# ufal/neuralmonkey

Measured on NVIDIA H100. Metric: train_target_tokens_per_sec, higher is better.
Workload: dtype f32 storage; tensor-core products in fp16 (vocabulary) / tf32 with fp32 accumulation

## Files before the change

neuralmonkey_b200/csrc/gru.cu:

```cuda
#include <stdlib.h>
#include <string.h>

#include "gemm_simt.cuh"
#include "gru_cluster.cuh"

namespace nm {

struct GruGatesEpi {
  const float* xproj;
  const float* hprev;
  float* gates;
  float* rh;
  int64_t T, H, t;
  __device__ void operator()(int64_t b, int64_t n, float acc) const {
    const int64_t base3 = (b * T + t) * 3 * H;
    const float g = sigmoidf_(acc + xproj[base3 + n]);
    gates[base3 + n] = g;
    if (n < H) rh[(b * T + t) * H + n] = g * hprev[(b * T + t) * H + n];
  }
};

struct GruCandEpi {
  const float* xproj;
  const float* hprev;
  float* gates;
  float* states;
  float* hnext;
  int64_t hnext_stride;
  const int32_t* lengths;
  const float* drop_mask;
  float* raw_states;
  int64_t T, H, t;
  __device__ void operator()(int64_t b, int64_t n, float acc) const {
    const int64_t base3 = (b * T + t) * 3 * H;
    const float c = tanhf(acc + xproj[base3 + 2 * H + n]);
    gates[base3 + 2 * H + n] = c;
    const float u = gates[base3 + H + n];
    const float h = hprev[(b * T + t) * H + n];
    const bool live = (lengths == nullptr) || (t < (int64_t)lengths[b]);
    float hn = live ? (u * h + (1.f - u) * c) : h;
    if (raw_states) raw_states[(b * T + t) * H + n] = live ? hn : 0.f;
    if (drop_mask && live) hn *= drop_mask[(b * T + t) * H + n];
    states[(b * T + t) * H + n] = live ? hn : 0.f;
    hnext[b * hnext_stride + n] = hn;
  }
};

__global__ void gru_bwd_gate_kernel(const float* __restrict__ gates, const float* __restrict__ hprev,
                                    const float* __restrict__ dstates, const float* __restrict__ dcarry,
                                    const int32_t* __restrict__ lengths,
                                    const float* __restrict__ drop_mask,
                                    const float* __restrict__ draw, float* __restrict__ dxproj,
                                    float* __restrict__ dhp, int64_t B, int64_t T, int64_t H,
                                    int64_t t) {
  const int64_t total = B * H;
  for (int64_t i = blockIdx.x * (int64_t)blockDim.x + threadIdx.x; i < total;
       i += (int64_t)gridDim.x * blockDim.x) {
    const int64_t b = i / H, n = i - b * H;
    const int64_t base3 = (b * T + t) * 3 * H, base1 = (b * T + t) * H;
    const bool live = (lengths == nullptr) || (t < (int64_t)lengths[b]);
    const float u = gates[base3 + H + n], c = gates[base3 + 2 * H + n];
    const float h = hprev[base1 + n];
    float dh = dcarry ? dcarry[i] : 0.f;
    if (!live) {
      dxproj[base3 + n] = 0.f;
      dxproj[base3 + H + n] = 0.f;
      dxproj[base3 + 2 * H + n] = 0.f;
      dhp[i] = dh;
      continue;
    }
    if (dstates) dh += dstates[base1 + n];
    if (drop_mask) dh *= drop_mask[base1 + n];
    if (draw) dh += draw[base1 + n];
    const float du = dh * (h - c);
    const float dc = dh * (1.f - u);
    dxproj[base3 + 2 * H + n] = dc * (1.f - c * c);
    dxproj[base3 + H + n] = du * u * (1.f - u);
    dhp[i] = dh * u;
  }
}

struct GruBwdCandEpi {
  const float* gates;
  const float* hprev;
  const int32_t* lengths;
  float* dxproj;
  float* dhp;
  int64_t T, H, t;
  __device__ void operator()(int64_t b, int64_t n, float drh) const {
    const bool live = (lengths == nullptr) || (t < (int64_t)lengths[b]);
    if (!live) return;
    const int64_t base3 = (b * T + t) * 3 * H;
    const float r = gates[base3 + n];
    const float h = hprev[(b * T + t) * H + n];
    dxproj[base3 + n] = drh * h * r * (1.f - r);
    dhp[b * H + n] += drh * r;
  }
};

struct GruBwdGatesEpi {
  const float* dhp;
  float* dcarry;
  int64_t H;
  __device__ void operator()(int64_t b, int64_t n, float acc) const {
    dcarry[b * H + n] = dhp[b * H + n] + acc;
  }
};

}

using namespace nm;

namespace {

bool cluster_path_ok(int64_t H) {
  static int forced = -1;
  if (forced < 0) {
    const char* e = getenv("NMB200_GRU");
    forced = (e && strcmp(e, "steps") == 0) ? 1 : 0;
  }
  return forced == 0 && H >= 8 && H <= 320;
}

int g_gru_mode = 0;

struct ClusterPlan {
  int Bc, nclusters, sl;
  size_t smem;
};

template <class Kern>
int max_active_clusters(Kern kern, size_t smem) {
  cudaLaunchConfig_t cfg = {};
  cfg.gridDim = dim3(GC_CLUSTER * 64);
  cfg.blockDim = dim3(GC_THREADS);
  cfg.dynamicSmemBytes = smem;
  cudaLaunchAttribute attr[1];
  attr[0].id = cudaLaunchAttributeClusterDimension;
  attr[0].val.clusterDim.x = GC_CLUSTER;
  attr[0].val.clusterDim.y = 1;
  attr[0].val.clusterDim.z = 1;
  cfg.attrs = attr;
  cfg.numAttrs = 1;
  int n = 0;
  if (cudaFuncSetAttribute(kern, cudaFuncAttributeMaxDynamicSharedMemorySize, GC_SMEM_CAP) != cudaSuccess ||
      cudaOccupancyMaxActiveClusters(&n, kern, &cfg) != cudaSuccess || n < 1) {
    cudaGetLastError();
    n = sm_count() / GC_CLUSTER / 2;
  }
  return n;
}

int resident_clusters(bool backward) {
  static int cached[2] = {0, 0};
  if (cached[backward] == 0)
    cached[backward] = backward ? max_active_clusters(gru_seq_bwd_cluster_kernel<GC_MAX_SL>, 128 * 1024)
                                : max_active_clusters(gru_seq_fwd_cluster_kernel<GC_MAX_SL>, 128 * 1024);
  return cached[backward];
}

ClusterPlan plan_clusters(int64_t B, int64_t H, int sm_budget, bool backward) {
  ClusterPlan p;
  p.sl = (int)((H + GC_SLICES - 1) / GC_SLICES);
  int max_clusters = resident_clusters(backward);
  if (sm_budget > 0 && sm_budget / GC_CLUSTER < max_clusters) max_clusters = sm_budget / GC_CLUSTER;
  if (max_clusters < 1) max_clusters = 1;
  int Bc = (int)((B + max_clusters - 1) / max_clusters);
  Bc = (Bc + 3) / 4 * 4;
  const size_t per_row = (size_t)(backward ? gc_bwd_row_floats(p.sl) : gc_fwd_row_floats(p.sl)) * 4;
  const int cap = (int)((GC_SMEM_CAP - GC_BAR_BYTES) / per_row) / 4 * 4;
  if (Bc > cap) Bc = cap;
  if (Bc < 4) Bc = 4;
  p.Bc = Bc;
  p.nclusters = (int)((B + Bc - 1) / Bc);
  p.smem = GC_BAR_BYTES + per_row * Bc;
  return p;
}

template <class Args, class Kern>
int launch_cluster(Kern kern, const Args& args, const ClusterPlan& p, cudaStream_t s, const char* name) {
  NM_CUDA_TRY(cudaFuncSetAttribute(kern, cudaFuncAttributeMaxDynamicSharedMemorySize, (int)p.smem));
  cudaLaunchConfig_t cfg = {};
  cfg.gridDim = dim3((unsigned)(p.nclusters * GC_CLUSTER));
  cfg.blockDim = dim3(GC_THREADS);
  cfg.dynamicSmemBytes = p.smem;
  cfg.stream = s;
  cudaLaunchAttribute attr[1];
  attr[0].id = cudaLaunchAttributeClusterDimension;
  attr[0].val.clusterDim.x = GC_CLUSTER;
  attr[0].val.clusterDim.y = 1;
  attr[0].val.clusterDim.z = 1;
  cfg.attrs = attr;
  cfg.numAttrs = 1;
  NM_CUDA_TRY(cudaLaunchKernelEx(&cfg, kern, args));
  NM_LAUNCH_CHECK(name);
  return NM_OK;
}

#define NM_GC_DISPATCH(KERN, args, plan, s, name)                  \
  switch ((plan).sl) {                                             \
    case 1: return launch_cluster(KERN<1>, args, plan, s, name);   \
    case 2: return launch_cluster(KERN<2>, args, plan, s, name);   \
    case 3: return launch_cluster(KERN<3>, args, plan, s, name);   \
    case 4: return launch_cluster(KERN<4>, args, plan, s, name);   \
    case 5: return launch_cluster(KERN<5>, args, plan, s, name);   \
    case 6: return launch_cluster(KERN<6>, args, plan, s, name);   \
    case 7: return launch_cluster(KERN<7>, args, plan, s, name);   \
    case 8: return launch_cluster(KERN<8>, args, plan, s, name);   \
    case 9: return launch_cluster(KERN<9>, args, plan, s, name);   \
    default: return launch_cluster(KERN<10>, args, plan, s, name); \
  }

}

extern "C" {

int nm_gru_resident_clusters(int backward) { return resident_clusters(backward != 0); }

int nm_gru_set_mode(int mode) {
  NM_REQUIRE(mode == 0 || mode == 1, NM_E_INVALID, "nm_gru_set_mode: mode must be 0 (tensor cores) or 1 (exact fp32)");
  g_gru_mode = mode;
  return NM_OK;
}

static long long* g_gru_prof = nullptr;
int nm_gru_debug_profile(void* counters) {
  g_gru_prof = reinterpret_cast<long long*>(counters);
  return NM_OK;
}

int nm_gru_seq_fwd(const float* xproj, const float* Wgh, const float* Wch, const float* h0,
                   const int32_t* lengths, const float* drop_mask, int reverse, float* states,
                   float* raw_states, float* final_state, float* gates, float* hprev, float* rh,
                   int64_t B, int64_t T, int64_t H, int sm_budget, void* stream) {
  NM_REQUIRE(xproj && Wgh && Wch && states && final_state && gates && hprev && rh, NM_E_INVALID,
             "nm_gru_seq_fwd: null pointer");
  NM_REQUIRE(B > 0 && T > 0 && H > 0, NM_E_INVALID, "nm_gru_seq_fwd: bad sizes B=%lld T=%lld H=%lld",
             (long long)B, (long long)T, (long long)H);
  cudaStream_t s = (cudaStream_t)stream;
  if (cluster_path_ok(H)) {
    GcFwdArgs a{xproj, Wgh, Wch, h0, lengths, drop_mask, states, raw_states, final_state, gates,
                hprev, rh, (int)B, (int)T, (int)H, 0, reverse, g_gru_prof};
    const ClusterPlan p = plan_clusters(B, H, sm_budget, false);
    a.Bc = p.Bc;
    NM_GC_DISPATCH(gru_seq_fwd_cluster_kernel, a, p, s, "nm_gru_seq_fwd(cluster)");
  }
  const int64_t t_first = reverse ? T - 1 : 0;
  if (h0)
    NM_CUDA_TRY(cudaMemcpy2DAsync(hprev + t_first * H, sizeof(float) * T * H, h0, sizeof(float) * H,
                                  sizeof(float) * H, B, cudaMemcpyDeviceToDevice, s));
  else
    NM_CUDA_TRY(cudaMemset2DAsync(hprev + t_first * H, sizeof(float) * T * H, 0, sizeof(float) * H, B, s));
  for (int64_t step = 0; step < T; ++step) {
    const int64_t t = reverse ? T - 1 - step : step;
    GruGatesEpi e1{xproj, hprev, gates, rh, T, H, t};
    simt_gemm_launch(hprev + t * H, T * H, 1, Wgh, 2 * H, 1, B, 2 * H, H, e1, s);
    const bool last = (step == T - 1);
    const int64_t t_next = reverse ? t - 1 : t + 1;
    GruCandEpi e2{xproj, hprev, gates, states, last ? final_state : hprev + t_next * H,
                  last ? H : T * H, lengths, drop_mask, raw_states, T, H, t};
    simt_gemm_launch(rh + t * H, T * H, 1, Wch, H, 1, B, H, H, e2, s);
  }
  count_launches(2 * T - 1);
  NM_LAUNCH_CHECK("nm_gru_seq_fwd");
  return NM_OK;
}

int nm_gru_seq_bwd(const float* Wgh, const float* Wch, const int32_t* lengths,
                   const float* drop_mask, int reverse, const float* gates, const float* hprev,
                   const float* dstates, const float* draw, const float* dfinal,
                   float* dxproj, float* dh0, float* work, int64_t B, int64_t T, int64_t H,
                   int sm_budget, void* stream) {
  NM_REQUIRE(Wgh && Wch && gates && hprev && dxproj && work, NM_E_INVALID,
             "nm_gru_seq_bwd: null pointer");
  NM_REQUIRE(B > 0 && T > 0 && H > 0, NM_E_INVALID, "nm_gru_seq_bwd: bad sizes");
  cudaStream_t s = (cudaStream_t)stream;
  if (cluster_path_ok(H)) {
    GcBwdArgs a{Wgh, Wch, lengths, drop_mask, gates, hprev, dstates, draw, dfinal, dxproj, dh0,
                (int)B, (int)T, (int)H, 0, reverse, g_gru_prof};
    const ClusterPlan p = plan_clusters(B, H, sm_budget, true);
    a.Bc = p.Bc;
    NM_GC_DISPATCH(gru_seq_bwd_cluster_kernel, a, p, s, "nm_gru_seq_bwd(cluster)");
  }
  float* dcarry = work;
  float* dhp = work + B * H;
  if (dfinal)
    NM_CUDA_TRY(cudaMemcpyAsync(dcarry, dfinal, sizeof(float) * B * H, cudaMemcpyDeviceToDevice, s));
  else
    NM_CUDA_TRY(cudaMemsetAsync(dcarry, 0, sizeof(float) * B * H, s));
  const int threads = 256;
  int64_t blocks = ceil_div(B * H, threads);
  const int64_t cap = (int64_t)sm_count() * 8;
  if (blocks > cap) blocks = cap;
  for (int64_t step = T - 1; step >= 0; --step) {
    const int64_t t = reverse ? T - 1 - step : step;
    gru_bwd_gate_kernel<<<(unsigned)blocks, threads, 0, s>>>(gates, hprev, dstates, dcarry, lengths,
                                                            drop_mask, draw, dxproj, dhp, B, T, H, t);
    GruBwdCandEpi g1{gates, hprev, lengths, dxproj, dhp, T, H, t};
    simt_gemm_launch(dxproj + t * 3 * H + 2 * H, T * 3 * H, 1, Wch, 1, H, B, H, H, g1, s);
    GruBwdGatesEpi g2{dhp, dcarry, H};
    simt_gemm_launch(dxproj + t * 3 * H, T * 3 * H, 1, Wgh, 1, 2 * H, B, H, 2 * H, g2, s);
  }
  if (dh0)
    NM_CUDA_TRY(cudaMemcpyAsync(dh0, dcarry, sizeof(float) * B * H, cudaMemcpyDeviceToDevice, s));
  count_launches(3 * T - 1);
  NM_LAUNCH_CHECK("nm_gru_seq_bwd");
  return NM_OK;
}


int nm_gru_seq_fwd_pair(const float* xproj_a, const float* Wgh_a, const float* Wch_a, int reverse_a,
                        float* states_a, float* final_a, float* gates_a, float* hprev_a, float* rh_a,
                        const float* xproj_b, const float* Wgh_b, const float* Wch_b, int reverse_b,
                        float* states_b, float* final_b, float* gates_b, float* hprev_b, float* rh_b,
                        const int32_t* lengths, int64_t B, int64_t T, int64_t H, void* stream) {
  NM_REQUIRE(xproj_a && Wgh_a && Wch_a && states_a && final_a && gates_a && hprev_a && rh_a && xproj_b &&
                 Wgh_b && Wch_b && states_b && final_b && gates_b && hprev_b && rh_b,
             NM_E_INVALID, "nm_gru_seq_fwd_pair: null pointer");
  NM_REQUIRE(B > 0 && T > 0 && H > 0, NM_E_INVALID, "nm_gru_seq_fwd_pair: bad sizes");
  int rc = nm_gru_seq_fwd(xproj_a, Wgh_a, Wch_a, nullptr, lengths, nullptr, reverse_a, states_a, nullptr, final_a,
                          gates_a, hprev_a, rh_a, B, T, H, 0, stream);
  if (rc) return rc;
  return nm_gru_seq_fwd(xproj_b, Wgh_b, Wch_b, nullptr, lengths, nullptr, reverse_b, states_b, nullptr, final_b,
                        gates_b, hprev_b, rh_b, B, T, H, 0, stream);
}

int nm_gru_seq_bwd_pair(const float* Wgh_a, const float* Wch_a, int reverse_a, const float* gates_a,
                        const float* hprev_a, const float* dstates_a, const float* dfinal_a, float* dxproj_a,
                        const float* Wgh_b, const float* Wch_b, int reverse_b, const float* gates_b,
                        const float* hprev_b, const float* dstates_b, const float* dfinal_b, float* dxproj_b,
                        const int32_t* lengths, float* work, int64_t B, int64_t T, int64_t H, void* stream) {
  NM_REQUIRE(Wgh_a && Wch_a && gates_a && hprev_a && dxproj_a && Wgh_b && Wch_b && gates_b && hprev_b &&
                 dxproj_b && work,
             NM_E_INVALID, "nm_gru_seq_bwd_pair: null pointer");
  NM_REQUIRE(B > 0 && T > 0 && H > 0, NM_E_INVALID, "nm_gru_seq_bwd_pair: bad sizes");
  int rc = nm_gru_seq_bwd(Wgh_a, Wch_a, lengths, nullptr, reverse_a, gates_a, hprev_a, dstates_a, nullptr, dfinal_a,
                          dxproj_a, nullptr, work, B, T, H, 0, stream);
  if (rc) return rc;
  return nm_gru_seq_bwd(Wgh_b, Wch_b, lengths, nullptr, reverse_b, gates_b, hprev_b, dstates_b, nullptr, dfinal_b,
                        dxproj_b, nullptr, work, B, T, H, 0, stream);
}

}
```

neuralmonkey_b200/csrc/gru_cluster.cuh:

```cuda
#pragma once
#include "common.cuh"

namespace nm {

constexpr int GC_CLUSTER = 8;
constexpr int GC_SLICES = 32;
constexpr int GC_UPW = 4;
constexpr int GC_WARPS = 10;
constexpr int GC_THREADS = GC_WARPS * 32;
constexpr int GC_MAX_UNITS = GC_WARPS * GC_UPW;
constexpr int GC_RB = 2;
constexpr int GC_MAX_SL = 10;
constexpr int GC_SMEM_CAP = 200 * 1024;
constexpr int GC_BAR_BYTES = 64;
constexpr int GC_XS = 4;
constexpr int GC_PF = 8;

__host__ __device__ constexpr int gc_row(int SL) { return GC_SLICES * 4 * (((SL + 3) / 4) | 1); }
__host__ __device__ constexpr int gc_fwd_row_floats(int SL) {
  return 3 * gc_row(SL) + GC_MAX_UNITS * (1 + 2 * GC_XS) + 1;
}
__host__ __device__ constexpr int gc_bwd_row_floats(int SL) {
  return 4 * gc_row(SL) + GC_MAX_UNITS * (1 + 2 * GC_PF) + 1;
}

template <int SL>
struct GcGeom {
  static constexpr int SLP = 4 * (((SL + 3) / 4) | 1);
  static constexpr int ROW = GC_SLICES * SLP;
  static __device__ __forceinline__ int pos(int j) { return (j / SL) * SLP + (j % SL); }
};

__device__ __forceinline__ void cluster_barrier() {
  asm volatile("barrier.cluster.arrive.release.aligned;\n\tbarrier.cluster.wait.acquire.aligned;" ::
                   : "memory");
}
__device__ __forceinline__ uint32_t cluster_rank() {
  uint32_t r;
  asm volatile("mov.u32 %0, %%cluster_ctarank;" : "=r"(r));
  return r;
}

__device__ __forceinline__ uint32_t gc_smem_u32(const void* p) {
  return (uint32_t)__cvta_generic_to_shared(p);
}
__device__ __forceinline__ void gc_mbar_init(uint32_t bar) {
  asm volatile("mbarrier.init.shared::cta.b64 [%0], 1;" ::"r"(bar));
  asm volatile("fence.mbarrier_init.release.cluster;" ::: "memory");
}
__device__ __forceinline__ void gc_mbar_arm(uint32_t bar, uint32_t bytes) {
  asm volatile("mbarrier.arrive.expect_tx.shared::cta.b64 _, [%0], %1;" ::"r"(bar), "r"(bytes) : "memory");
}
__device__ __forceinline__ void gc_mbar_wait(uint32_t bar, uint32_t parity) {
  uint32_t done;
  do {
    asm volatile(
        "{\n\t.reg .pred p;\n\t"
        "mbarrier.try_wait.parity.acquire.cluster.shared::cta.b64 p, [%1], %2;\n\t"
        "selp.u32 %0, 1, 0, p;\n\t}"
        : "=r"(done)
        : "r"(bar), "r"(parity)
        : "memory");
  } while (!done);
}
__device__ __forceinline__ void gc_send(uint32_t addr, uint32_t bar, uint32_t dst, float v) {
  uint32_t ra, rb;
  asm volatile("mapa.shared::cluster.u32 %0, %1, %2;" : "=r"(ra) : "r"(addr), "r"(dst));
  asm volatile("mapa.shared::cluster.u32 %0, %1, %2;" : "=r"(rb) : "r"(bar), "r"(dst));
  asm volatile("st.async.shared::cluster.mbarrier::complete_tx::bytes.b32 [%0], %1, [%2];" ::"r"(ra),
               "r"(__float_as_uint(v)), "r"(rb)
               : "memory");
}

__device__ __forceinline__ void cp_async4(float* smem_dst, const float* gmem_src) {
  const uint32_t d = gc_smem_u32(smem_dst);
  asm volatile("cp.async.ca.shared.global [%0], [%1], 4;" ::"r"(d), "l"(gmem_src) : "memory");
}
__device__ __forceinline__ void cp_async_commit() { asm volatile("cp.async.commit_group;" ::: "memory"); }
__device__ __forceinline__ void cp_async_wait_all() { asm volatile("cp.async.wait_all;" ::: "memory"); }

template <int N, int O>
__device__ __forceinline__ void gc_reduce_level(float (&v)[N], int lane) {
  constexpr int n = N * O / 16;
  if constexpr (n > 1) {
    const bool upper = (lane & O) != 0;
#pragma unroll
    for (int i = 0; i < n / 2; ++i) {
      const float keep = upper ? v[i + n / 2] : v[i];
      const float send = upper ? v[i] : v[i + n / 2];
      v[i] = keep + __shfl_xor_sync(0xffffffffu, send, O);
    }
  } else {
    v[0] += __shfl_xor_sync(0xffffffffu, v[0], O);
  }
  if constexpr (O > 1) gc_reduce_level<N, O / 2>(v, lane);
}
template <int N>
__device__ __forceinline__ void gc_reduce_scatter(float (&v)[N], int lane) {
  gc_reduce_level<N, 16>(v, lane);
}

template <int SL>
__device__ __forceinline__ void gc_dot(const float* __restrict__ vec, int row0, int lane,
                                       const float (&w)[GC_UPW][SL], float (&acc)[GC_RB][GC_UPW]) {
#pragma unroll
  for (int r = 0; r < GC_RB; ++r)
#pragma unroll
    for (int u = 0; u < GC_UPW; ++u) acc[r][u] = 0.f;
  const float* base = vec + row0 * GcGeom<SL>::ROW + lane * GcGeom<SL>::SLP;
#pragma unroll
  for (int c = 0; c < SL; c += 4) {
    const int n = SL - c < 4 ? SL - c : 4;
#pragma unroll
    for (int r = 0; r < GC_RB; ++r) {
      const float* p = base + r * GcGeom<SL>::ROW + c;
      float x[4];
      if (n == 4) {
        const float4 q = *reinterpret_cast<const float4*>(p);
        x[0] = q.x; x[1] = q.y; x[2] = q.z; x[3] = q.w;
      } else {
        if (n >= 2) {
          const float2 q = *reinterpret_cast<const float2*>(p);
          x[0] = q.x; x[1] = q.y;
        }
        if (n == 1) x[0] = p[0];
        if (n == 3) x[2] = p[2];
      }
#pragma unroll
      for (int u = 0; u < GC_UPW; ++u)
#pragma unroll
        for (int i = 0; i < 4; ++i)
          if (i < n) acc[r][u] = fmaf(x[i], w[u][c + i], acc[r][u]);
    }
  }
}

template <int SL>
__device__ __forceinline__ void gc_load_w(float (&w)[GC_UPW][SL], const float* __restrict__ W,
                                          int64_t sk, int64_t su, int unit0, int unit_limit, int k0, int H) {
#pragma unroll
  for (int u = 0; u < GC_UPW; ++u)
#pragma unroll
    for (int i = 0; i < SL; ++i) {
      const int unit = unit0 + u, k = k0 + i;
      const bool ok = (unit < unit_limit) && (k < H);
      w[u][i] = ok ? W[(int64_t)k * sk + (int64_t)unit * su] : 0.f;
    }
}

struct GcProf {
  bool on;
  unsigned t0;
  __device__ __forceinline__ explicit GcProf(const long long* out)
      : on(out != nullptr && blockIdx.x == 0 && threadIdx.x == 0), t0(on ? (unsigned)clock() : 0u) {}
  __device__ __forceinline__ void lap(long long* out, int slot) {
    if (on) {
      const unsigned t1 = (unsigned)clock();
      out[slot] += (long long)(t1 - t0);
      t0 = t1;
    }
  }
};

struct GcFwdArgs {
  const float* xproj;
  const float* Wgh;
  const float* Wch;
  const float* h0;
  const int32_t* lengths;
  const float* drop_mask;
  float* states;
  float* raw_states;
  float* final_state;
  float* gates;
  float* hprev;
  float* rh;
  int B, T, H, Bc, reverse;
  long long* prof;
};

__device__ __forceinline__ void gc_fwd_prefetch(const GcFwdArgs& a, int t, float* dst, int b0, int nrows,
                                                int ubeg, int UW) {
  const int H = a.H, T = a.T;
  for (int idx = threadIdx.x; idx < a.Bc * UW; idx += GC_THREADS) {
    const int b = idx / UW, ul = idx - b * UW, j = ubeg + ul;
    if (b < nrows && j < H) {
      const int64_t row = ((int64_t)(b0 + b) * T + t);
      const float* xp = a.xproj + row * 3 * H + j;
      float* xd = dst + (b * GC_MAX_UNITS + ul) * GC_XS;
      cp_async4(xd, xp);
      cp_async4(xd + 1, xp + H);
      cp_async4(xd + 2, xp + 2 * H);
      if (a.drop_mask) cp_async4(xd + 3, a.drop_mask + row * H + j);
    }
  }
  cp_async_commit();
}

__device__ __forceinline__ uint32_t gc_phase_bytes(const GcFwdArgs& a) { return (uint32_t)(a.Bc * a.H * 4); }

template <int SL>
__global__ void __launch_bounds__(GC_THREADS, 1) gru_seq_fwd_cluster_kernel(GcFwdArgs a) {
  extern __shared__ __align__(16) float gc_smem[];
  constexpr int ROW = GcGeom<SL>::ROW;
  const int H = a.H, T = a.T, Bc = a.Bc;
  float* hbuf = gc_smem + GC_BAR_BYTES / 4;
  float* rhbuf = hbuf + 2 * Bc * ROW;
  float* us = rhbuf + Bc * ROW;
  float* xs = us + Bc * GC_MAX_UNITS;
  int* lens = reinterpret_cast<int*>(xs + 2 * Bc * GC_MAX_UNITS * GC_XS);
  const uint32_t bar_h = gc_smem_u32(gc_smem), bar_rh = bar_h + 16;

  const int rank = (int)cluster_rank();
  const int ubeg = rank * H / GC_CLUSTER;
  const int unit_limit = (rank + 1) * H / GC_CLUSTER;
  const int UW = unit_limit - ubeg;
  const int b0 = (blockIdx.x / GC_CLUSTER) * Bc;
  const int nrows = min(Bc, a.B - b0);
  const int lane = threadIdx.x & 31, warp = threadIdx.x >> 5;
  const int unit0_local = warp * GC_UPW;
  const int unit0 = ubeg + unit0_local;
  const bool warp_live = unit0 < unit_limit;

  float wr[GC_UPW][SL], wu[GC_UPW][SL], wc[GC_UPW][SL];
  gc_load_w<SL>(wr, a.Wgh, 2 * H, 1, unit0, unit_limit, lane * SL, H);
  gc_load_w<SL>(wu, a.Wgh + H, 2 * H, 1, unit0, unit_limit, lane * SL, H);
  gc_load_w<SL>(wc, a.Wch, H, 1, unit0, unit_limit, lane * SL, H);

  const int g1 = lane >> 4, r1 = (lane >> 3) & 1, u1 = (lane >> 1) & 3;
  const int r2 = (lane >> 4) & 1, u2 = (lane >> 2) & 3, copy2 = lane & 3;
  const int copy1 = ((lane >> 4) << 1) | (lane & 1);
  const bool ok1 = unit0 + u1 < unit_limit, ok2 = unit0 + u2 < unit_limit;
  const int j1 = unit0 + u1, j2 = unit0 + u2;
  const int pos1 = ok1 ? GcGeom<SL>::pos(j1) : 0, pos2 = ok2 ? GcGeom<SL>::pos(j2) : 0;

  if (threadIdx.x == 0) {
    gc_mbar_init(bar_h);
    gc_mbar_init(bar_h + 8);
    gc_mbar_init(bar_rh);
    gc_mbar_arm(bar_h, gc_phase_bytes(a));
    gc_mbar_arm(bar_h + 8, gc_phase_bytes(a));
    gc_mbar_arm(bar_rh, gc_phase_bytes(a));
  }
  for (int i = threadIdx.x; i < 3 * Bc * ROW; i += GC_THREADS) hbuf[i] = 0.f;
  for (int i = threadIdx.x; i < 2 * Bc * GC_MAX_UNITS * GC_XS; i += GC_THREADS) xs[i] = 0.f;
  for (int b = threadIdx.x; b < Bc; b += GC_THREADS)
    lens[b] = b < nrows ? (a.lengths ? a.lengths[b0 + b] : T) : 0;


  __syncthreads();
  cluster_barrier();
  const int t_first = a.reverse ? T - 1 : 0;
  for (int idx = threadIdx.x; idx < Bc * UW; idx += GC_THREADS) {
    const int b = idx / UW, j = ubeg + (idx - b * UW);
    const float hv = (b < nrows && a.h0) ? a.h0[(int64_t)(b0 + b) * H + j] : 0.f;
    if (b < nrows) a.hprev[((int64_t)(b0 + b) * T + t_first) * H + j] = hv;
    const uint32_t addr = gc_smem_u32(hbuf + b * ROW + GcGeom<SL>::pos(j));
    for (int d = 0; d < GC_CLUSTER; ++d) gc_send(addr, bar_h, d, hv);
  }
  gc_fwd_prefetch(a, t_first, xs, b0, nrows, ubeg, UW);

  GcProf prof(a.prof);
  for (int step = 0; step < T; ++step) {
    const int t = a.reverse ? T - 1 - step : step;
    const bool last = (step == T - 1);
    const int t_next = a.reverse ? t - 1 : t + 1;
    const int64_t row0 = (int64_t)b0 * T + t;
    const int par = step & 1;
    const float* hb = hbuf + par * Bc * ROW;
    const float* xc = xs + par * Bc * GC_MAX_UNITS * GC_XS;

    gc_mbar_wait(bar_h + 8 * par, (step >> 1) & 1);
    if (threadIdx.x == 0 && step + 2 < T) gc_mbar_arm(bar_h + 8 * par, gc_phase_bytes(a));
    prof.lap(a.prof, 0);
    cp_async_wait_all();
    __syncthreads();
    if (!last) gc_fwd_prefetch(a, t_next, xs + (par ^ 1) * Bc * GC_MAX_UNITS * GC_XS, b0, nrows, ubeg, UW);
    prof.lap(a.prof, 1);

    if (warp_live) {
      for (int r0 = 0; r0 < Bc; r0 += GC_RB) {
        float ar[GC_RB][GC_UPW], au[GC_RB][GC_UPW];
        gc_dot<SL>(hb, r0, lane, wr, ar);
        gc_dot<SL>(hb, r0, lane, wu, au);
        float v[2 * GC_RB * GC_UPW];
#pragma unroll
        for (int r = 0; r < GC_RB; ++r)
#pragma unroll
          for (int u = 0; u < GC_UPW; ++u) {
            v[r * GC_UPW + u] = ar[r][u];
            v[GC_RB * GC_UPW + r * GC_UPW + u] = au[r][u];
          }
        gc_reduce_scatter<2 * GC_RB * GC_UPW>(v, lane);
        const int b = r0 + r1, ul = unit0_local + u1;
        const float g = sigmoidf_(v[0] + xc[(b * GC_MAX_UNITS + ul) * GC_XS + g1]);
        const float rhv = g * hb[b * ROW + pos1];
        const float rh_peer = __shfl_xor_sync(0xffffffffu, rhv, 16);
        const float rh_send = g1 == 0 ? rhv : rh_peer;
        if (ok1) {
          if ((lane & 1) == 0) {
            if (b < nrows) {
              const int64_t row = row0 + (int64_t)b * T;
              a.gates[row * 3 * H + g1 * H + j1] = g;
              if (g1 == 0) a.rh[row * H + j1] = rhv;
            }
            if (g1 == 1) us[b * GC_MAX_UNITS + ul] = g;
          }
          const uint32_t addr = gc_smem_u32(rhbuf + b * ROW + pos1);
          gc_send(addr, bar_rh, 2 * copy1, rh_send);
          gc_send(addr, bar_rh, 2 * copy1 + 1, rh_send);
        }
      }
      __syncwarp();
    }
    prof.lap(a.prof, 2);
    gc_mbar_wait(bar_rh, step & 1);
    if (threadIdx.x == 0 && !last) gc_mbar_arm(bar_rh, gc_phase_bytes(a));
    prof.lap(a.prof, 3);

    if (warp_live) {
      const uint32_t bar_next = bar_h + 8 * (par ^ 1);
      float* hn_buf = hbuf + (par ^ 1) * Bc * ROW;
      for (int r0 = 0; r0 < Bc; r0 += GC_RB) {
        float ac[GC_RB][GC_UPW];
        gc_dot<SL>(rhbuf, r0, lane, wc, ac);
        float v[GC_RB * GC_UPW];
#pragma unroll
        for (int r = 0; r < GC_RB; ++r)
#pragma unroll
          for (int u = 0; u < GC_UPW; ++u) v[r * GC_UPW + u] = ac[r][u];
        gc_reduce_scatter<GC_RB * GC_UPW>(v, lane);
        if (!ok2) continue;
        const int b = r0 + r2, ul = unit0_local + u2;
        const float* xd = xc + (b * GC_MAX_UNITS + ul) * GC_XS;
        const float c = tanhf(v[0] + xd[2]);
        const float hv = hb[b * ROW + pos2];
        const float uu = us[b * GC_MAX_UNITS + ul];
        const bool live = t < lens[b];
        float hn = live ? (uu * hv + (1.f - uu) * c) : hv;
        const float raw = live ? hn : 0.f;
        if (a.drop_mask && live) hn *= xd[3];
        if (b < nrows) {
          const int64_t row = row0 + (int64_t)b * T;
          if (copy2 == 0) a.gates[row * 3 * H + 2 * H + j2] = c;
          else if (copy2 == 1) a.states[row * H + j2] = live ? hn : 0.f;
          else if (copy2 == 2) { if (a.raw_states) a.raw_states[row * H + j2] = raw; }
          else if (last) a.final_state[(int64_t)(b0 + b) * H + j2] = hn;
          else a.hprev[((int64_t)(b0 + b) * T + t_next) * H + j2] = hn;
        }
        if (!last) {
          const uint32_t addr = gc_smem_u32(hn_buf + b * ROW + pos2);
          gc_send(addr, bar_next, 2 * copy2, hn);
          gc_send(addr, bar_next, 2 * copy2 + 1, hn);
        }
      }
    }
    prof.lap(a.prof, 4);
  }
  cluster_barrier();
}

struct GcBwdArgs {
  const float* Wgh;
  const float* Wch;
  const int32_t* lengths;
  const float* drop_mask;
  const float* gates;
  const float* hprev;
  const float* dstates;
  const float* draw;
  const float* dfinal;
  float* dxproj;
  float* dh0;
  int B, T, H, Bc, reverse;
  long long* prof;
};

__device__ __forceinline__ float gc_bwd_e1(const GcBwdArgs& a, const float* pf, float dh, bool live,
                                           float& zc, float& zu) {
  if (!live) {
    zc = zu = 0.f;
    return dh;
  }
  const float uu = pf[1], c = pf[2], hv = pf[3];
  if (a.dstates) dh += pf[4];
  if (a.drop_mask) dh *= pf[5];
  if (a.draw) dh += pf[6];
  const float du = dh * (hv - c);
  const float dc = dh * (1.f - uu);
  zc = dc * (1.f - c * c);
  zu = du * uu * (1.f - uu);
  return dh * uu;
}

__device__ __forceinline__ void gc_bwd_prefetch(const GcBwdArgs& a, int t, float* dst, const int* lens, int b0,
                                                int ubeg, int UW) {
  const int H = a.H, T = a.T;
  for (int idx = threadIdx.x; idx < a.Bc * UW; idx += GC_THREADS) {
    const int b = idx / UW, u = idx - b * UW, j = ubeg + u;
    if (t >= lens[b]) continue;
    const int64_t row = (int64_t)(b0 + b) * T + t;
    float* d = dst + (b * GC_MAX_UNITS + u) * GC_PF;
    const float* g = a.gates + row * 3 * H + j;
    cp_async4(d, g);
    cp_async4(d + 1, g + H);
    cp_async4(d + 2, g + 2 * H);
    cp_async4(d + 3, a.hprev + row * H + j);
    if (a.dstates) cp_async4(d + 4, a.dstates + row * H + j);
    if (a.drop_mask) cp_async4(d + 5, a.drop_mask + row * H + j);
    if (a.draw) cp_async4(d + 6, a.draw + row * H + j);
  }
  cp_async_commit();
}

template <int SL>
__global__ void __launch_bounds__(GC_THREADS, 1) gru_seq_bwd_cluster_kernel(GcBwdArgs a) {
  extern __shared__ __align__(16) float gc_smem[];
  constexpr int ROW = GcGeom<SL>::ROW;
  const int H = a.H, T = a.T, Bc = a.Bc;
  float* vc = gc_smem + GC_BAR_BYTES / 4;
  float* vu = vc + Bc * ROW;
  float* vr = vu + 2 * Bc * ROW;
  float* dhp = vr + Bc * ROW;
  float* pf = dhp + Bc * GC_MAX_UNITS;
  int* lens = reinterpret_cast<int*>(pf + 2 * Bc * GC_MAX_UNITS * GC_PF);
  const uint32_t bar_a = gc_smem_u32(gc_smem), bar_b = bar_a + 16;
  const uint32_t bytes_a = (uint32_t)(2 * Bc * H * 4), bytes_b = (uint32_t)(Bc * H * 4);

  const int rank = (int)cluster_rank();
  const int ubeg = rank * H / GC_CLUSTER;
  const int unit_limit = (rank + 1) * H / GC_CLUSTER;
  const int UW = unit_limit - ubeg;
  const int b0 = (blockIdx.x / GC_CLUSTER) * Bc;
  const int nrows = min(Bc, a.B - b0);
  const int lane = threadIdx.x & 31, warp = threadIdx.x >> 5;
  const int unit0_local = warp * GC_UPW;
  const int unit0 = ubeg + unit0_local;
  const bool warp_live = unit0 < unit_limit;

  float w1[GC_UPW][SL], w2r[GC_UPW][SL], w2u[GC_UPW][SL];
  gc_load_w<SL>(w1, a.Wch, 1, H, unit0, unit_limit, lane * SL, H);
  gc_load_w<SL>(w2r, a.Wgh, 1, 2 * H, unit0, unit_limit, lane * SL, H);
  gc_load_w<SL>(w2u, a.Wgh + H, 1, 2 * H, unit0, unit_limit, lane * SL, H);

  const int rr_ = (lane >> 4) & 1, uq = (lane >> 2) & 3, copy = lane & 3;
  const bool ok = unit0 + uq < unit_limit;
  const int ji = unit0 + uq, ul = unit0_local + uq;
  const int pos = ok ? GcGeom<SL>::pos(ji) : 0;
  auto time_of = [reverse = a.reverse, T](int k) { return reverse ? k : T - 1 - k; };

  if (threadIdx.x == 0) {
    gc_mbar_init(bar_a);
    gc_mbar_init(bar_a + 8);
    gc_mbar_init(bar_b);
    gc_mbar_arm(bar_a, bytes_a);
    gc_mbar_arm(bar_a + 8, bytes_a);
    gc_mbar_arm(bar_b, bytes_b);
  }
  for (int i = threadIdx.x; i < 4 * Bc * ROW; i += GC_THREADS) vc[i] = 0.f;
  for (int i = threadIdx.x; i < 2 * Bc * GC_MAX_UNITS * GC_PF; i += GC_THREADS) pf[i] = 0.f;
  for (int b = threadIdx.x; b < Bc; b += GC_THREADS)
    lens[b] = b < nrows ? (a.lengths ? a.lengths[b0 + b] : T) : 0;
  __syncthreads();


  gc_bwd_prefetch(a, time_of(0), pf, lens, b0, ubeg, UW);
  cp_async_wait_all();
  __syncthreads();
  cluster_barrier();
  {
    const int t = time_of(0);
    for (int idx = threadIdx.x; idx < Bc * UW; idx += GC_THREADS) {
      const int b = idx / UW, u = idx - b * UW, j = ubeg + u;
      const bool live = t < lens[b];
      const float dh = (a.dfinal && b < nrows) ? a.dfinal[(int64_t)(b0 + b) * H + j] : 0.f;
      float zc, zu;
      dhp[b * GC_MAX_UNITS + u] = gc_bwd_e1(a, pf + (b * GC_MAX_UNITS + u) * GC_PF, dh, live, zc, zu);
      if (b < nrows) {
        const int64_t row = (int64_t)(b0 + b) * T + t;
        a.dxproj[row * 3 * H + H + j] = zu;
        a.dxproj[row * 3 * H + 2 * H + j] = zc;
      }
      const int p = GcGeom<SL>::pos(j);
      const uint32_t ac = gc_smem_u32(vc + b * ROW + p), au = gc_smem_u32(vu + b * ROW + p);
      for (int d = 0; d < GC_CLUSTER; ++d) {
        gc_send(ac, bar_a, d, zc);
        gc_send(au, bar_a, d, zu);
      }
    }
  }

  GcProf prof(a.prof);
  for (int k = 0; k < T; ++k) {
    const int t = time_of(k);
    const bool last = (k == T - 1);
    const int64_t row0 = (int64_t)b0 * T + t;
    const int par = k & 1;
    const float* pfc = pf + par * Bc * GC_MAX_UNITS * GC_PF;
    float* pfn = pf + (par ^ 1) * Bc * GC_MAX_UNITS * GC_PF;

    gc_mbar_wait(bar_a + 8 * par, (k >> 1) & 1);
    if (threadIdx.x == 0 && k + 2 < T) gc_mbar_arm(bar_a + 8 * par, bytes_a);
    prof.lap(a.prof, 0);
    __syncthreads();
    if (!last) gc_bwd_prefetch(a, time_of(k + 1), pfn, lens, b0, ubeg, UW);
    prof.lap(a.prof, 1);

    if (warp_live) {
      for (int r0 = 0; r0 < Bc; r0 += GC_RB) {
        float acc[GC_RB][GC_UPW];
        gc_dot<SL>(vc, r0, lane, w1, acc);
        float v[GC_RB * GC_UPW];
#pragma unroll
        for (int r = 0; r < GC_RB; ++r)
#pragma unroll
          for (int u = 0; u < GC_UPW; ++u) v[r * GC_UPW + u] = acc[r][u];
        gc_reduce_scatter<GC_RB * GC_UPW>(v, lane);
        if (!ok) continue;
        const int b = r0 + rr_;
        const float drh = v[0];
        const bool live = t < lens[b];
        const float* s = pfc + (b * GC_MAX_UNITS + ul) * GC_PF;
        const float rg = s[0], hv = s[3];
        const float zr = live ? drh * hv * rg * (1.f - rg) : 0.f;
        if (copy == 0) {
          if (b < nrows) a.dxproj[(row0 + (int64_t)b * T) * 3 * H + ji] = zr;
          if (live) dhp[b * GC_MAX_UNITS + ul] += drh * rg;
        }
        const uint32_t addr = gc_smem_u32(vr + b * ROW + pos);
        gc_send(addr, bar_b, 2 * copy, zr);
        gc_send(addr, bar_b, 2 * copy + 1, zr);
      }
      __syncwarp();
    }
    prof.lap(a.prof, 2);
    gc_mbar_wait(bar_b, k & 1);
    if (threadIdx.x == 0 && !last) gc_mbar_arm(bar_b, bytes_b);
    prof.lap(a.prof, 3);
    cp_async_wait_all();
    __syncthreads();
    prof.lap(a.prof, 4);

    if (warp_live) {
      const float* vuc = vu + par * Bc * ROW;
      const int tn = last ? t : time_of(k + 1);
      for (int r0 = 0; r0 < Bc; r0 += GC_RB) {
        float accr[GC_RB][GC_UPW], accu[GC_RB][GC_UPW];
        gc_dot<SL>(vr, r0, lane, w2r, accr);
        gc_dot<SL>(vuc, r0, lane, w2u, accu);
        float v[GC_RB * GC_UPW];
#pragma unroll
        for (int r = 0; r < GC_RB; ++r)
#pragma unroll
          for (int u = 0; u < GC_UPW; ++u) v[r * GC_UPW + u] = accr[r][u] + accu[r][u];
        gc_reduce_scatter<GC_RB * GC_UPW>(v, lane);
        const int b = r0 + rr_;
        const float dcarry = ok ? dhp[b * GC_MAX_UNITS + ul] + v[0] : 0.f;
        __syncwarp();
        if (!ok) continue;
        if (last) {
          if (a.dh0 && copy == 0 && b < nrows) a.dh0[(int64_t)(b0 + b) * H + ji] = dcarry;
          continue;
        }
        float zc, zu;
        const float d = gc_bwd_e1(a, pfn + (b * GC_MAX_UNITS + ul) * GC_PF, dcarry, tn < lens[b], zc, zu);
        if (b < nrows) {
          const int64_t row = (int64_t)(b0 + b) * T + tn;
          if (copy == 1) a.dxproj[row * 3 * H + H + ji] = zu;
          else if (copy == 2) a.dxproj[row * 3 * H + 2 * H + ji] = zc;
        }
        if (copy == 0) dhp[b * GC_MAX_UNITS + ul] = d;
        const uint32_t ac = gc_smem_u32(vc + b * ROW + pos);
        const uint32_t au = gc_smem_u32(vu + ((par ^ 1) * Bc + b) * ROW + pos);
        const uint32_t bar_next = bar_a + 8 * (par ^ 1);
        gc_send(ac, bar_next, 2 * copy, zc);
        gc_send(ac, bar_next, 2 * copy + 1, zc);
        gc_send(au, bar_next, 2 * copy, zu);
        gc_send(au, bar_next, 2 * copy + 1, zu);
      }
    }
    prof.lap(a.prof, 5);
  }
  cluster_barrier();
}

}
```

Before: 1.016 million.

## Stage update-gate weights in shared memory and widen row batching in cluster GRU

Moves the update-gate recurrent weight slice from registers into shared memory, which frees registers so each warp can process four batch rows per dot step instead of two. The forward gate dot products are fused so one pass over the hidden state feeds both the reset and update gates. Lane-to-output mapping and the cluster broadcast pattern are reorganised so each lane sends to four peer CTAs, and the shared-memory cap and batch-chunk rounding are adjusted to fit the staged weights. The cost is extra shared-memory traffic for weight reads, smaller possible batch chunks, and more sends per lane.

```diff
diff --git a/neuralmonkey_b200/csrc/gru.cu b/neuralmonkey_b200/csrc/gru.cu
--- a/neuralmonkey_b200/csrc/gru.cu
+++ b/neuralmonkey_b200/csrc/gru.cu
@@ -166,14 +166,14 @@
   if (sm_budget > 0 && sm_budget / GC_CLUSTER < max_clusters) max_clusters = sm_budget / GC_CLUSTER;
   if (max_clusters < 1) max_clusters = 1;
   int Bc = (int)((B + max_clusters - 1) / max_clusters);
-  Bc = (Bc + 3) / 4 * 4;
+  Bc = (Bc + 1) / 2 * 2;
   const size_t per_row = (size_t)(backward ? gc_bwd_row_floats(p.sl) : gc_fwd_row_floats(p.sl)) * 4;
-  const int cap = (int)((GC_SMEM_CAP - GC_BAR_BYTES) / per_row) / 4 * 4;
+  const size_t fixed = GC_BAR_BYTES + (size_t)(gc_w_floats(p.sl) + GC_PAD_ROWS * gc_row(p.sl)) * 4;
+  const int cap = (int)((GC_SMEM_CAP - fixed) / per_row) / 2 * 2;
   if (Bc > cap) Bc = cap;
-  if (Bc < 4) Bc = 4;
   p.Bc = Bc;
   p.nclusters = (int)((B + Bc - 1) / Bc);
-  p.smem = GC_BAR_BYTES + per_row * Bc;
+  p.smem = fixed + per_row * Bc;
   return p;
 }
 
diff --git a/neuralmonkey_b200/csrc/gru_cluster.cuh b/neuralmonkey_b200/csrc/gru_cluster.cuh
--- a/neuralmonkey_b200/csrc/gru_cluster.cuh
+++ b/neuralmonkey_b200/csrc/gru_cluster.cuh
@@ -9,12 +9,13 @@
 constexpr int GC_WARPS = 10;
 constexpr int GC_THREADS = GC_WARPS * 32;
 constexpr int GC_MAX_UNITS = GC_WARPS * GC_UPW;
-constexpr int GC_RB = 2;
+constexpr int GC_RB = 4;
 constexpr int GC_MAX_SL = 10;
-constexpr int GC_SMEM_CAP = 200 * 1024;
+constexpr int GC_SMEM_CAP = 227 * 1024;
 constexpr int GC_BAR_BYTES = 64;
 constexpr int GC_XS = 4;
 constexpr int GC_PF = 8;
+constexpr int GC_PAD_ROWS = 2;
 
 __host__ __device__ constexpr int gc_row(int SL) { return GC_SLICES * 4 * (((SL + 3) / 4) | 1); }
 __host__ __device__ constexpr int gc_fwd_row_floats(int SL) {
@@ -23,6 +24,7 @@
 __host__ __device__ constexpr int gc_bwd_row_floats(int SL) {
   return 4 * gc_row(SL) + GC_MAX_UNITS * (1 + 2 * GC_PF) + 1;
 }
+__host__ __device__ constexpr int gc_w_floats(int SL) { return GC_MAX_UNITS * GC_SLICES * 4 * ((SL + 3) / 4); }
 
 template <int SL>
 struct GcGeom {
@@ -65,8 +67,8 @@
 }
 __device__ __forceinline__ void gc_send(uint32_t addr, uint32_t bar, uint32_t dst, float v) {
   uint32_t ra, rb;
-  asm volatile("mapa.shared::cluster.u32 %0, %1, %2;" : "=r"(ra) : "r"(addr), "r"(dst));
-  asm volatile("mapa.shared::cluster.u32 %0, %1, %2;" : "=r"(rb) : "r"(bar), "r"(dst));
+  asm("mapa.shared::cluster.u32 %0, %1, %2;" : "=r"(ra) : "r"(addr), "r"(dst));
+  asm("mapa.shared::cluster.u32 %0, %1, %2;" : "=r"(rb) : "r"(bar), "r"(dst));
   asm volatile("st.async.shared::cluster.mbarrier::complete_tx::bytes.b32 [%0], %1, [%2];" ::"r"(ra),
                "r"(__float_as_uint(v)), "r"(rb)
                : "memory");
@@ -100,11 +102,25 @@
   gc_reduce_level<N, 16>(v, lane);
 }
 
-template <int SL>
+__device__ __forceinline__ void gc_load_chunk(const float* p, int n, float (&x)[4]) {
+  if (n == 4) {
+    const float4 q = *reinterpret_cast<const float4*>(p);
+    x[0] = q.x; x[1] = q.y; x[2] = q.z; x[3] = q.w;
+  } else {
+    if (n >= 2) {
+      const float2 q = *reinterpret_cast<const float2*>(p);
+      x[0] = q.x; x[1] = q.y;
+    }
+    if (n == 1) x[0] = p[0];
+    if (n == 3) x[2] = p[2];
+  }
+}
+
+template <int SL, int RB>
 __device__ __forceinline__ void gc_dot(const float* __restrict__ vec, int row0, int lane,
-                                       const float (&w)[GC_UPW][SL], float (&acc)[GC_RB][GC_UPW]) {
-#pragma unroll
-  for (int r = 0; r < GC_RB; ++r)
+                                       const float (&w)[GC_UPW][SL], float (&acc)[RB][GC_UPW]) {
+#pragma unroll
+  for (int r = 0; r < RB; ++r)
 #pragma unroll
     for (int u = 0; u < GC_UPW; ++u) acc[r][u] = 0.f;
   const float* base = vec + row0 * GcGeom<SL>::ROW + lane * GcGeom<SL>::SLP;
@@ -112,25 +128,73 @@
   for (int c = 0; c < SL; c += 4) {
     const int n = SL - c < 4 ? SL - c : 4;
 #pragma unroll
-    for (int r = 0; r < GC_RB; ++r) {
-      const float* p = base + r * GcGeom<SL>::ROW + c;
+    for (int r = 0; r < RB; ++r) {
       float x[4];
-      if (n == 4) {
-        const float4 q = *reinterpret_cast<const float4*>(p);
-        x[0] = q.x; x[1] = q.y; x[2] = q.z; x[3] = q.w;
-      } else {
-        if (n >= 2) {
-          const float2 q = *reinterpret_cast<const float2*>(p);
-          x[0] = q.x; x[1] = q.y;
-        }
-        if (n == 1) x[0] = p[0];
-        if (n == 3) x[2] = p[2];
-      }
+      gc_load_chunk(base + r * GcGeom<SL>::ROW + c, n, x);
 #pragma unroll
       for (int u = 0; u < GC_UPW; ++u)
 #pragma unroll
         for (int i = 0; i < 4; ++i)
           if (i < n) acc[r][u] = fmaf(x[i], w[u][c + i], acc[r][u]);
+    }
+  }
+}
+
+template <int SL, int RB>
+__device__ __forceinline__ void gc_dot_smem_add(const float* __restrict__ vec, int row0, int lane,
+                                                const float* __restrict__ ws, float (&acc)[RB][GC_UPW]) {
+  constexpr int NC = (SL + 3) / 4;
+  const float* base = vec + row0 * GcGeom<SL>::ROW + lane * GcGeom<SL>::SLP;
+#pragma unroll
+  for (int c = 0; c < SL; c += 4) {
+    const int n = SL - c < 4 ? SL - c : 4;
+    float w[GC_UPW][4];
+#pragma unroll
+    for (int u = 0; u < GC_UPW; ++u) {
+      const float4 q = reinterpret_cast<const float4*>(ws)[(u * NC + c / 4) * GC_SLICES + lane];
+      w[u][0] = q.x; w[u][1] = q.y; w[u][2] = q.z; w[u][3] = q.w;
+    }
+#pragma unroll
+    for (int r = 0; r < RB; ++r) {
+      float x[4];
+      gc_load_chunk(base + r * GcGeom<SL>::ROW + c, n, x);
+#pragma unroll
+      for (int u = 0; u < GC_UPW; ++u)
+#pragma unroll
+        for (int i = 0; i < 4; ++i)
+          if (i < n) acc[r][u] = fmaf(x[i], w[u][i], acc[r][u]);
+    }
+  }
+}
+
+template <int SL, int RB>
+__device__ __forceinline__ void gc_dot2(const float* __restrict__ vec, int row0, int lane,
+                                        const float (&w)[GC_UPW][SL], const float* __restrict__ ws,
+                                        float (&accr)[RB][GC_UPW], float (&accu)[RB][GC_UPW]) {
+  constexpr int NC = (SL + 3) / 4;
+#pragma unroll
+  for (int r = 0; r < RB; ++r)
+#pragma unroll
+    for (int u = 0; u < GC_UPW; ++u) accr[r][u] = accu[r][u] = 0.f;
+  const float* base = vec + row0 * GcGeom<SL>::ROW + lane * GcGeom<SL>::SLP;
+#pragma unroll
+  for (int c = 0; c < SL; c += 4) {
+    const int n = SL - c < 4 ? SL - c : 4;
+    float x[RB][4];
+#pragma unroll
+    for (int r = 0; r < RB; ++r) gc_load_chunk(base + r * GcGeom<SL>::ROW + c, n, x[r]);
+#pragma unroll
+    for (int u = 0; u < GC_UPW; ++u) {
+      const float4 q = reinterpret_cast<const float4*>(ws)[(u * NC + c / 4) * GC_SLICES + lane];
+      const float wu[4] = {q.x, q.y, q.z, q.w};
+#pragma unroll
+      for (int r = 0; r < RB; ++r)
+#pragma unroll
+        for (int i = 0; i < 4; ++i)
+          if (i < n) {
+            accr[r][u] = fmaf(x[r][i], w[u][c + i], accr[r][u]);
+            accu[r][u] = fmaf(x[r][i], wu[i], accu[r][u]);
+          }
     }
   }
 }
@@ -145,6 +209,17 @@
       const int unit = unit0 + u, k = k0 + i;
       const bool ok = (unit < unit_limit) && (k < H);
       w[u][i] = ok ? W[(int64_t)k * sk + (int64_t)unit * su] : 0.f;
+    }
+}
+template <int SL>
+__device__ __forceinline__ void gc_stage_w(float* ws, const float* __restrict__ W, int64_t sk, int64_t su,
+                                           int unit0, int unit_limit, int lane, int H) {
+  constexpr int NC = (SL + 3) / 4;
+  for (int u = 0; u < GC_UPW; ++u)
+    for (int i = 0; i < 4 * NC; ++i) {
+      const int unit = unit0 + u, k = lane * SL + i;
+      const bool ok = (unit < unit_limit) && (i < SL) && (k < H);
+      ws[((u * NC + i / 4) * GC_SLICES + lane) * 4 + i % 4] = ok ? W[(int64_t)k * sk + (int64_t)unit * su] : 0.f;
     }
 }
 
@@ -182,6 +257,7 @@
 __device__ __forceinline__ void gc_fwd_prefetch(const GcFwdArgs& a, int t, float* dst, int b0, int nrows,
                                                 int ubeg, int UW) {
   const int H = a.H, T = a.T;
+#pragma unroll 1
   for (int idx = threadIdx.x; idx < a.Bc * UW; idx += GC_THREADS) {
     const int b = idx / UW, ul = idx - b * UW, j = ubeg + ul;
     if (b < nrows && j < H) {
@@ -204,7 +280,8 @@
   extern __shared__ __align__(16) float gc_smem[];
   constexpr int ROW = GcGeom<SL>::ROW;
   const int H = a.H, T = a.T, Bc = a.Bc;
-  float* hbuf = gc_smem + GC_BAR_BYTES / 4;
+  float* wsu = gc_smem + GC_BAR_BYTES / 4;
+  float* hbuf = wsu + gc_w_floats(SL);
   float* rhbuf = hbuf + 2 * Bc * ROW;
   float* us = rhbuf + Bc * ROW;
   float* xs = us + Bc * GC_MAX_UNITS;
@@ -221,18 +298,17 @@
   const int unit0_local = warp * GC_UPW;
   const int unit0 = ubeg + unit0_local;
   const bool warp_live = unit0 < unit_limit;
-
-  float wr[GC_UPW][SL], wu[GC_UPW][SL], wc[GC_UPW][SL];
+  float* wsu_warp = wsu + warp * (gc_w_floats(SL) / GC_WARPS);
+
+  float wr[GC_UPW][SL], wc[GC_UPW][SL];
+  gc_stage_w<SL>(wsu_warp, a.Wgh + H, 2 * H, 1, unit0, unit_limit, lane, H);
   gc_load_w<SL>(wr, a.Wgh, 2 * H, 1, unit0, unit_limit, lane * SL, H);
-  gc_load_w<SL>(wu, a.Wgh + H, 2 * H, 1, unit0, unit_limit, lane * SL, H);
   gc_load_w<SL>(wc, a.Wch, H, 1, unit0, unit_limit, lane * SL, H);
 
-  const int g1 = lane >> 4, r1 = (lane >> 3) & 1, u1 = (lane >> 1) & 3;
-  const int r2 = (lane >> 4) & 1, u2 = (lane >> 2) & 3, copy2 = lane & 3;
-  const int copy1 = ((lane >> 4) << 1) | (lane & 1);
-  const bool ok1 = unit0 + u1 < unit_limit, ok2 = unit0 + u2 < unit_limit;
-  const int j1 = unit0 + u1, j2 = unit0 + u2;
-  const int pos1 = ok1 ? GcGeom<SL>::pos(j1) : 0, pos2 = ok2 ? GcGeom<SL>::pos(j2) : 0;
+  const int g1 = lane >> 4, r1 = (lane >> 2) & 3, ul1 = unit0_local + (lane & 3);
+  const int r2 = (lane >> 3) & 3, ul2 = unit0_local + ((lane >> 1) & 3), copy2 = lane & 1;
+  const bool ok1 = ubeg + ul1 < unit_limit, ok2 = ubeg + ul2 < unit_limit;
+  const int pos1 = ok1 ? GcGeom<SL>::pos(ubeg + ul1) : 0, pos2 = ok2 ? GcGeom<SL>::pos(ubeg + ul2) : 0;
 
   if (threadIdx.x == 0) {
     gc_mbar_init(bar_h);
@@ -279,10 +355,10 @@
     prof.lap(a.prof, 1);
 
     if (warp_live) {
+#pragma unroll 1
       for (int r0 = 0; r0 < Bc; r0 += GC_RB) {
         float ar[GC_RB][GC_UPW], au[GC_RB][GC_UPW];
-        gc_dot<SL>(hb, r0, lane, wr, ar);
-        gc_dot<SL>(hb, r0, lane, wu, au);
+        gc_dot2<SL, GC_RB>(hb, r0, lane, wr, wsu_warp, ar, au);
         float v[2 * GC_RB * GC_UPW];
 #pragma unroll
         for (int r = 0; r < GC_RB; ++r)
@@ -292,24 +368,23 @@
             v[GC_RB * GC_UPW + r * GC_UPW + u] = au[r][u];
           }
         gc_reduce_scatter<2 * GC_RB * GC_UPW>(v, lane);
-        const int b = r0 + r1, ul = unit0_local + u1;
-        const float g = sigmoidf_(v[0] + xc[(b * GC_MAX_UNITS + ul) * GC_XS + g1]);
+        const int b = r0 + r1;
+        const bool ok = ok1 && b < Bc;
+        const int j1 = ubeg + ul1;
+        const float g = ok ? sigmoidf_(v[0] + xc[(b * GC_MAX_UNITS + ul1) * GC_XS + g1]) : 0.f;
         const float rhv = g * hb[b * ROW + pos1];
         const float rh_peer = __shfl_xor_sync(0xffffffffu, rhv, 16);
-        const float rh_send = g1 == 0 ? rhv : rh_peer;
-        if (ok1) {
-          if ((lane & 1) == 0) {
-            if (b < nrows) {
-              const int64_t row = row0 + (int64_t)b * T;
-              a.gates[row * 3 * H + g1 * H + j1] = g;
-              if (g1 == 0) a.rh[row * H + j1] = rhv;
-            }
-            if (g1 == 1) us[b * GC_MAX_UNITS + ul] = g;
-          }
-          const uint32_t addr = gc_smem_u32(rhbuf + b * ROW + pos1);
-          gc_send(addr, bar_rh, 2 * copy1, rh_send);
-          gc_send(addr, bar_rh, 2 * copy1 + 1, rh_send);
+        if (!ok) continue;
+        if (g1 == 1) us[b * GC_MAX_UNITS + ul1] = g;
+        if (b < nrows) {
+          const int64_t row = row0 + (int64_t)b * T;
+          a.gates[row * 3 * H + g1 * H + j1] = g;
+          if (g1 == 0) a.rh[row * H + j1] = rhv;
         }
+        const float sv = g1 == 0 ? rhv : rh_peer;
+        const uint32_t addr = gc_smem_u32(rhbuf + b * ROW + pos1);
+#pragma unroll
+        for (int d = 0; d < GC_CLUSTER / 2; ++d) gc_send(addr, bar_rh, g1 * (GC_CLUSTER / 2) + d, sv);
       }
       __syncwarp();
     }
@@ -321,37 +396,42 @@
     if (warp_live) {
       const uint32_t bar_next = bar_h + 8 * (par ^ 1);
       float* hn_buf = hbuf + (par ^ 1) * Bc * ROW;
+#pragma unroll 1
       for (int r0 = 0; r0 < Bc; r0 += GC_RB) {
-        float ac[GC_RB][GC_UPW];
-        gc_dot<SL>(rhbuf, r0, lane, wc, ac);
+        float acc[GC_RB][GC_UPW];
+        gc_dot<SL, GC_RB>(rhbuf, r0, lane, wc, acc);
         float v[GC_RB * GC_UPW];
 #pragma unroll
         for (int r = 0; r < GC_RB; ++r)
 #pragma unroll
-          for (int u = 0; u < GC_UPW; ++u) v[r * GC_UPW + u] = ac[r][u];
+          for (int u = 0; u < GC_UPW; ++u) v[r * GC_UPW + u] = acc[r][u];
         gc_reduce_scatter<GC_RB * GC_UPW>(v, lane);
-        if (!ok2) continue;
-        const int b = r0 + r2, ul = unit0_local + u2;
-        const float* xd = xc + (b * GC_MAX_UNITS + ul) * GC_XS;
+        const int b = r0 + r2;
+        if (!ok2 || b >= Bc) continue;
+        const int j2 = ubeg + ul2;
+        const float* xd = xc + (b * GC_MAX_UNITS + ul2) * GC_XS;
         const float c = tanhf(v[0] + xd[2]);
         const float hv = hb[b * ROW + pos2];
-        const float uu = us[b * GC_MAX_UNITS + ul];
+        const float uu = us[b * GC_MAX_UNITS + ul2];
         const bool live = t < lens[b];
         float hn = live ? (uu * hv + (1.f - uu) * c) : hv;
         const float raw = live ? hn : 0.f;
         if (a.drop_mask && live) hn *= xd[3];
         if (b < nrows) {
           const int64_t row = row0 + (int64_t)b * T;
-          if (copy2 == 0) a.gates[row * 3 * H + 2 * H + j2] = c;
-          else if (copy2 == 1) a.states[row * H + j2] = live ? hn : 0.f;
-          else if (copy2 == 2) { if (a.raw_states) a.raw_states[row * H + j2] = raw; }
-          else if (last) a.final_state[(int64_t)(b0 + b) * H + j2] = hn;
-          else a.hprev[((int64_t)(b0 + b) * T + t_next) * H + j2] = hn;
+          if (copy2 == 0) {
+            a.gates[row * 3 * H + 2 * H + j2] = c;
+            a.states[row * H + j2] = live ? hn : 0.f;
+          } else {
+            if (a.raw_states) a.raw_states[row * H + j2] = raw;
+            if (last) a.final_state[(int64_t)(b0 + b) * H + j2] = hn;
+            else a.hprev[((int64_t)(b0 + b) * T + t_next) * H + j2] = hn;
+          }
         }
         if (!last) {
           const uint32_t addr = gc_smem_u32(hn_buf + b * ROW + pos2);
-          gc_send(addr, bar_next, 2 * copy2, hn);
-          gc_send(addr, bar_next, 2 * copy2 + 1, hn);
+#pragma unroll
+          for (int d = 0; d < GC_CLUSTER / 2; ++d) gc_send(addr, bar_next, copy2 * (GC_CLUSTER / 2) + d, hn);
         }
       }
     }
@@ -396,6 +476,7 @@
 __device__ __forceinline__ void gc_bwd_prefetch(const GcBwdArgs& a, int t, float* dst, const int* lens, int b0,
                                                 int ubeg, int UW) {
   const int H = a.H, T = a.T;
+#pragma unroll 1
   for (int idx = threadIdx.x; idx < a.Bc * UW; idx += GC_THREADS) {
     const int b = idx / UW, u = idx - b * UW, j = ubeg + u;
     if (t >= lens[b]) continue;
@@ -418,7 +499,8 @@
   extern __shared__ __align__(16) float gc_smem[];
   constexpr int ROW = GcGeom<SL>::ROW;
   const int H = a.H, T = a.T, Bc = a.Bc;
-  float* vc = gc_smem + GC_BAR_BYTES / 4;
+  float* wsu = gc_smem + GC_BAR_BYTES / 4;
+  float* vc = wsu + gc_w_floats(SL);
   float* vu = vc + Bc * ROW;
   float* vr = vu + 2 * Bc * ROW;
   float* dhp = vr + Bc * ROW;
@@ -437,16 +519,18 @@
   const int unit0_local = warp * GC_UPW;
   const int unit0 = ubeg + unit0_local;
   const bool warp_live = unit0 < unit_limit;
-
-  float w1[GC_UPW][SL], w2r[GC_UPW][SL], w2u[GC_UPW][SL];
+  float* wsu_warp = wsu + warp * (gc_w_floats(SL) / GC_WARPS);
+
+  float w1[GC_UPW][SL], w2r[GC_UPW][SL];
+  gc_stage_w<SL>(wsu_warp, a.Wgh + H, 1, 2 * H, unit0, unit_limit, lane, H);
   gc_load_w<SL>(w1, a.Wch, 1, H, unit0, unit_limit, lane * SL, H);
   gc_load_w<SL>(w2r, a.Wgh, 1, 2 * H, unit0, unit_limit, lane * SL, H);
-  gc_load_w<SL>(w2u, a.Wgh + H, 1, 2 * H, unit0, unit_limit, lane * SL, H);
-
-  const int rr_ = (lane >> 4) & 1, uq = (lane >> 2) & 3, copy = lane & 3;
-  const bool ok = unit0 + uq < unit_limit;
-  const int ji = unit0 + uq, ul = unit0_local + uq;
+
+  const int rq = (lane >> 3) & 3, ul = unit0_local + ((lane >> 1) & 3), copy = lane & 1;
+  const int ji = ubeg + ul;
+  const bool ok = ji < unit_limit;
   const int pos = ok ? GcGeom<SL>::pos(ji) : 0;
+
   auto time_of = [reverse = a.reverse, T](int k) { return reverse ? k : T - 1 - k; };
 
   if (threadIdx.x == 0) {
@@ -507,17 +591,18 @@
     prof.lap(a.prof, 1);
 
     if (warp_live) {
+#pragma unroll 1
       for (int r0 = 0; r0 < Bc; r0 += GC_RB) {
         float acc[GC_RB][GC_UPW];
-        gc_dot<SL>(vc, r0, lane, w1, acc);
+        gc_dot<SL, GC_RB>(vc, r0, lane, w1, acc);
         float v[GC_RB * GC_UPW];
 #pragma unroll
         for (int r = 0; r < GC_RB; ++r)
 #pragma unroll
           for (int u = 0; u < GC_UPW; ++u) v[r * GC_UPW + u] = acc[r][u];
         gc_reduce_scatter<GC_RB * GC_UPW>(v, lane);
-        if (!ok) continue;
-        const int b = r0 + rr_;
+        const int b = r0 + rq;
+        if (!ok || b >= Bc) continue;
         const float drh = v[0];
         const bool live = t < lens[b];
         const float* s = pfc + (b * GC_MAX_UNITS + ul) * GC_PF;
@@ -528,8 +613,8 @@
           if (live) dhp[b * GC_MAX_UNITS + ul] += drh * rg;
         }
         const uint32_t addr = gc_smem_u32(vr + b * ROW + pos);
-        gc_send(addr, bar_b, 2 * copy, zr);
-        gc_send(addr, bar_b, 2 * copy + 1, zr);
+#pragma unroll
+        for (int d = 0; d < GC_CLUSTER / 2; ++d) gc_send(addr, bar_b, copy * (GC_CLUSTER / 2) + d, zr);
       }
       __syncwarp();
     }
@@ -544,39 +629,41 @@
     if (warp_live) {
       const float* vuc = vu + par * Bc * ROW;
       const int tn = last ? t : time_of(k + 1);
+      const uint32_t bar_next = bar_a + 8 * (par ^ 1);
+#pragma unroll 1
       for (int r0 = 0; r0 < Bc; r0 += GC_RB) {
-        float accr[GC_RB][GC_UPW], accu[GC_RB][GC_UPW];
-        gc_dot<SL>(vr, r0, lane, w2r, accr);
-        gc_dot<SL>(vuc, r0, lane, w2u, accu);
+        float acc[GC_RB][GC_UPW];
+        gc_dot<SL, GC_RB>(vr, r0, lane, w2r, acc);
+        gc_dot_smem_add<SL, GC_RB>(vuc, r0, lane, wsu_warp, acc);
         float v[GC_RB * GC_UPW];
 #pragma unroll
         for (int r = 0; r < GC_RB; ++r)
 #pragma unroll
-          for (int u = 0; u < GC_UPW; ++u) v[r * GC_UPW + u] = accr[r][u] + accu[r][u];
+          for (int u = 0; u < GC_UPW; ++u) v[r * GC_UPW + u] = acc[r][u];
         gc_reduce_scatter<GC_RB * GC_UPW>(v, lane);
-        const int b = r0 + rr_;
-        const float dcarry = ok ? dhp[b * GC_MAX_UNITS + ul] + v[0] : 0.f;
+        const int b = r0 + rq;
+        const bool okb = ok && b < Bc;
+        const float dcarry = okb ? dhp[b * GC_MAX_UNITS + ul] + v[0] : 0.f;
         __syncwarp();
-        if (!ok) continue;
+        if (!okb) continue;
         if (last) {
           if (a.dh0 && copy == 0 && b < nrows) a.dh0[(int64_t)(b0 + b) * H + ji] = dcarry;
           continue;
         }
         float zc, zu;
         const float d = gc_bwd_e1(a, pfn + (b * GC_MAX_UNITS + ul) * GC_PF, dcarry, tn < lens[b], zc, zu);
+        if (copy == 0) dhp[b * GC_MAX_UNITS + ul] = d;
         if (b < nrows) {
           const int64_t row = (int64_t)(b0 + b) * T + tn;
-          if (copy == 1) a.dxproj[row * 3 * H + H + ji] = zu;
-          else if (copy == 2) a.dxproj[row * 3 * H + 2 * H + ji] = zc;
+          a.dxproj[row * 3 * H + (2 - copy) * H + ji] = copy == 0 ? zc : zu;
         }
-        if (copy == 0) dhp[b * GC_MAX_UNITS + ul] = d;
         const uint32_t ac = gc_smem_u32(vc + b * ROW + pos);
         const uint32_t au = gc_smem_u32(vu + ((par ^ 1) * Bc + b) * ROW + pos);
-        const uint32_t bar_next = bar_a + 8 * (par ^ 1);
-        gc_send(ac, bar_next, 2 * copy, zc);
-        gc_send(ac, bar_next, 2 * copy + 1, zc);
-        gc_send(au, bar_next, 2 * copy, zu);
-        gc_send(au, bar_next, 2 * copy + 1, zu);
+#pragma unroll
+        for (int d2 = 0; d2 < GC_CLUSTER / 2; ++d2) {
+          gc_send(ac, bar_next, copy * (GC_CLUSTER / 2) + d2, zc);
+          gc_send(au, bar_next, copy * (GC_CLUSTER / 2) + d2, zu);
+        }
       }
     }
     prof.lap(a.prof, 5);
```

Measured after the change: 1.072 million (median of 6 runs). +5.5%, better.
